# Schatten2021/rust-raytracing

Measured on AMD Instinct MI355X. Metric: Mrays/s (primary rays, whole node), 10k-sphere 1080p 64spp, higher is better.
Workload: dtype f64; 1 GPU; C2: 10k random spheres (scene seed 1), 1920x1080, 64 spp; width=1920, height=1080, rays_per_pixel=64, n_objects=10000, partition=single GPU

## Files before the change

### rust-raytracing_amd/csrc/rtx_bvh.h

```cpp
#pragma once

#include <hip/hip_runtime.h>
#include <stdint.h>

#include <algorithm>
#include <cmath>
#include <cstring>
#include <numeric>
#include <vector>

namespace rtx {

struct BvhNode {
    float lo[3];
    uint32_t link;
    float hi[3];
    uint32_t count;
};
static_assert(sizeof(BvhNode) == 32, "BvhNode must be 32 bytes");

constexpr uint32_t kBvhTriLeaf = 0x10000u;
constexpr int kBvhLeafSize = 1;
constexpr int kBvhTriLeafMax = 8;

struct BvhBox { double lo[3], hi[3]; };

struct BvhBuild {
    std::vector<BvhNode> nodes;
    std::vector<uint32_t> prims;
    std::vector<uint32_t> tri_order;
    std::vector<uint8_t> flat;
    bool has_spheres = false, has_tris = false;
    double origin_limit = 0.0;
    double abs_pad = 0.0;
};

inline float round_down_f32(double x)
{
    float f = (float)x;
    if ((double)f > x) f = std::nextafterf(f, -INFINITY);
    return f;
}

inline float round_up_f32(double x)
{
    float f = (float)x;
    if ((double)f < x) f = std::nextafterf(f, INFINITY);
    return f;
}

inline bool sphere_box(const double s[4], BvhBox &b)
{
    const double r = std::fabs(s[3]);
    for (int a = 0; a < 3; ++a) {
        if (!std::isfinite(s[a]) || !std::isfinite(r)) return false;
        const double pad = (std::fabs(s[a]) + r) * (1.0 / 1048576.0) + 1e-300;
        b.lo[a] = s[a] - r - pad;
        b.hi[a] = s[a] + r + pad;
    }
    return true;
}

inline bool triangle_footprint(const double v[9], BvhBox &b, int free_axis = 2)
{
    for (int a = 0; a < 3; ++a) {
        if (a == free_axis) { b.lo[a] = -INFINITY; b.hi[a] = INFINITY; continue; }
        const double x0 = v[a], x1 = v[3 + a], x2 = v[6 + a];
        if (!std::isfinite(x0) || !std::isfinite(x1) || !std::isfinite(x2)) return false;
        const double lo = std::fmin(x0, std::fmin(x1, x2)), hi = std::fmax(x0, std::fmax(x1, x2));
        const double pad = std::fmax(std::fabs(lo), std::fabs(hi)) * (1.0 / 1048576.0) + 1e-300;
        b.lo[a] = lo - pad;
        b.hi[a] = hi + pad;
    }
    return true;
}

#ifndef RTX_BVH_SAH_BINS
#define RTX_BVH_SAH_BINS 16
#endif
constexpr int kBvhSahBins = RTX_BVH_SAH_BINS;
constexpr int kBvhSahExtraDepth = 6;

inline void bvh_append_tree(const std::vector<BvhBox> &box, int dims, uint32_t leaf_size, uint32_t leaf_flag,
                            BvhBuild &out, std::vector<uint32_t> &order_out, bool use_sah = true, int free_axis = 2,
                            uint32_t order_base = 0)
{
    const uint32_t n = (uint32_t)box.size();
    const int ax[3] = { dims == 2 && free_axis == 0 ? 1 : 0, dims == 2 && free_axis != 2 ? 2 : 1, 2 };
    std::vector<double> cen((size_t)dims * n);
    for (uint32_t i = 0; i < n; ++i)
        for (int a = 0; a < dims; ++a) cen[(size_t)dims * i + a] = 0.5 * (box[i].lo[ax[a]] + box[i].hi[ax[a]]);
    std::vector<uint32_t> order(n);
    std::iota(order.begin(), order.end(), 0u);
    int balanced_depth = 1;
    for (uint64_t c = leaf_size; c < n; c *= 2) ++balanced_depth;
    const int max_depth = balanced_depth + kBvhSahExtraDepth;
    auto measure = [dims, &ax](const BvhBox &b) {
        const double dx = b.hi[ax[0]] - b.lo[ax[0]], dy = b.hi[ax[1]] - b.lo[ax[1]];
        if (dims == 2) return dx + dy;
        const double dz = b.hi[2] - b.lo[2];
        return dx * dy + dy * dz + dz * dx;
    };
    auto grow = [](BvhBox &b, const BvhBox &o) {
        for (int a = 0; a < 3; ++a) { b.lo[a] = std::min(b.lo[a], o.lo[a]); b.hi[a] = std::max(b.hi[a], o.hi[a]); }
    };
    auto empty_box = [] {
        BvhBox b;
        for (int a = 0; a < 3; ++a) { b.lo[a] = INFINITY; b.hi[a] = -INFINITY; }
        return b;
    };
    struct Task { uint32_t begin, end; int parent; int depth; };
    std::vector<Task> todo;
    todo.push_back({0u, n, -1, 1});
    while (!todo.empty()) {
        const Task t = todo.back();
        todo.pop_back();
        const uint32_t me = (uint32_t)out.nodes.size();
        if (t.parent >= 0) out.nodes[(size_t)t.parent].link = me;
        BvhBox b = empty_box();
        double clo[3], chi[3];
        for (int a = 0; a < 3; ++a) { clo[a] = INFINITY; chi[a] = -INFINITY; }
        for (uint32_t k = t.begin; k < t.end; ++k) {
            const uint32_t i = order[k];
            grow(b, box[i]);
            for (int a = 0; a < dims; ++a) {
                clo[a] = std::min(clo[a], cen[(size_t)dims * i + a]); chi[a] = std::max(chi[a], cen[(size_t)dims * i + a]);
            }
        }
        BvhNode node;
        for (int a = 0; a < 3; ++a) {
            node.lo[a] = round_down_f32(b.lo[a] - out.abs_pad);
            node.hi[a] = round_up_f32(b.hi[a] + out.abs_pad);
        }
        const uint32_t cnt = t.end - t.begin;
        if (cnt <= leaf_size) {
            node.link = (uint32_t)order_out.size();
            node.count = cnt | leaf_flag;
            for (uint32_t k = t.begin; k < t.end; ++k) order_out.push_back(order_base + order[k]);
            out.nodes.push_back(node);
            continue;
        }
        uint32_t mid = 0;
        bool sah_allowed = use_sah && cnt > 2;
        if (sah_allowed) {
            int need = 1;
            for (uint64_t c = leaf_size; c < cnt; c *= 2) ++need;
            sah_allowed = t.depth + need < max_depth;
        }
        if (sah_allowed) {
            double best_cost = INFINITY;
            int best_axis = -1, best_bin = -1;
            for (int a = 0; a < dims; ++a) {
                const double ext = chi[a] - clo[a];
                if (!(ext > 0.0)) continue;
                BvhBox bin_box[kBvhSahBins];
                uint32_t bin_cnt[kBvhSahBins];
                for (int k = 0; k < kBvhSahBins; ++k) { bin_box[k] = empty_box(); bin_cnt[k] = 0; }
                const double scale = (double)kBvhSahBins / ext;
                for (uint32_t k = t.begin; k < t.end; ++k) {
                    const uint32_t i = order[k];
                    int bi = (int)((cen[(size_t)dims * i + a] - clo[a]) * scale);
                    bi = bi < 0 ? 0 : (bi >= kBvhSahBins ? kBvhSahBins - 1 : bi);
                    grow(bin_box[bi], box[i]);
                    bin_cnt[bi] += 1;
                }
                double right_m[kBvhSahBins];
                uint32_t right_n[kBvhSahBins];
                BvhBox acc = empty_box();
                uint32_t accn = 0;
                for (int k = kBvhSahBins - 1; k >= 1; --k) {
                    if (bin_cnt[k]) grow(acc, bin_box[k]);
                    accn += bin_cnt[k];
                    right_m[k] = accn ? measure(acc) : 0.0;
                    right_n[k] = accn;
                }
                acc = empty_box();
                accn = 0;
                for (int k = 0; k + 1 < kBvhSahBins; ++k) {
                    if (bin_cnt[k]) grow(acc, bin_box[k]);
                    accn += bin_cnt[k];
                    if (accn == 0 || right_n[k + 1] == 0) continue;
                    const double cost = measure(acc) * accn + right_m[k + 1] * right_n[k + 1];
                    if (cost < best_cost) { best_cost = cost; best_axis = a; best_bin = k; }
                }
            }
            if (best_axis >= 0) {
                const double ext = chi[best_axis] - clo[best_axis];
                const double scale = (double)kBvhSahBins / ext;
                auto in_left = [&](uint32_t i) {
                    int bi = (int)((cen[(size_t)dims * i + best_axis] - clo[best_axis]) * scale);
                    bi = bi < 0 ? 0 : (bi >= kBvhSahBins ? kBvhSahBins - 1 : bi);
                    return bi <= best_bin;
                };
                mid = (uint32_t)(std::stable_partition(order.begin() + t.begin, order.begin() + t.end, in_left) - order.begin());
            }
        }
        if (mid <= t.begin || mid >= t.end) {
            int axis = 0;
            for (int a = 1; a < dims; ++a)
                if (chi[a] - clo[a] > chi[axis] - clo[axis]) axis = a;
            mid = t.begin + cnt / 2;
            std::nth_element(order.begin() + t.begin, order.begin() + mid, order.begin() + t.end,
                             [&](uint32_t x, uint32_t y) {
                                 const double cx = cen[(size_t)dims * x + axis], cy = cen[(size_t)dims * y + axis];
                                 return cx < cy || (cx == cy && x < y);
                             });
        }
        node.link = 0;
        node.count = 0;
        out.nodes.push_back(node);
        todo.push_back({mid, t.end, (int)me, t.depth + 1});
        todo.push_back({t.begin, mid, -1, t.depth + 1});
    }
}

inline BvhBuild build_bvh(const std::vector<BvhBox> &sphere_boxes, const std::vector<BvhBox> (&tri_boxes)[3], uint32_t tri_leaf_size,
                          bool use_sah = true)
{
    BvhBuild out;
    const bool want_s = !sphere_boxes.empty();
    const size_t n_tri = tri_boxes[0].size() + tri_boxes[1].size() + tri_boxes[2].size();
    if (!want_s && n_tri == 0) return out;
    double scale = 0.0;
    auto grow_scale = [&](const std::vector<BvhBox> &v) {
        for (const BvhBox &b : v)
            for (int a = 0; a < 3; ++a) {
                if (std::isfinite(b.lo[a])) scale = std::max(scale, std::fabs(b.lo[a]));
                if (std::isfinite(b.hi[a])) scale = std::max(scale, std::fabs(b.hi[a]));
            }
    };
    grow_scale(sphere_boxes);
    for (const auto &v : tri_boxes) grow_scale(v);
    out.origin_limit = 4.0 * scale + 1.0;
    out.abs_pad = out.origin_limit * (1.0 / 4194304.0);
    if (!(out.origin_limit < 1.0e28)) return BvhBuild();
    if (sphere_boxes.size() + n_tri >= 0x10000000ull) return BvhBuild();
    if (tri_leaf_size < 1) tri_leaf_size = 1;
    if (tri_leaf_size > (uint32_t)kBvhTriLeafMax) tri_leaf_size = (uint32_t)kBvhTriLeafMax;
    out.nodes.reserve(2 * (sphere_boxes.size() + n_tri) + 8);
    struct Sub { const std::vector<BvhBox> *boxes; int free_axis; uint32_t base; };
    std::vector<Sub> subs;
    if (want_s) subs.push_back({&sphere_boxes, -1, 0u});
    uint32_t base = 0;
    for (int f = 2; f >= 0; --f) {
        if (!tri_boxes[f].empty()) subs.push_back({&tri_boxes[f], f, base});
        base += (uint32_t)tri_boxes[f].size();
    }
    std::vector<uint32_t> joints;
    for (size_t k = 0; k < subs.size(); ++k) {
        if (k + 1 < subs.size()) {
            joints.push_back((uint32_t)out.nodes.size());
            out.nodes.emplace_back();
        } else if (!joints.empty()) {
            out.nodes[joints.back()].link = (uint32_t)out.nodes.size();
        }
        if (k > 0 && k + 1 < subs.size()) out.nodes[joints[k - 1]].link = joints[k];
        const size_t first = out.nodes.size();
        if (subs[k].free_axis < 0) {
            bvh_append_tree(*subs[k].boxes, 3, (uint32_t)kBvhLeafSize, 0u, out, out.prims, use_sah);
            out.has_spheres = true;
        } else {
            bvh_append_tree(*subs[k].boxes, 2, tri_leaf_size, kBvhTriLeaf, out, out.tri_order, use_sah, subs[k].free_axis, subs[k].base);
            out.has_tris = true;
        }
        out.flat.resize(out.nodes.size(), 0);
        if (subs[k].free_axis == 2) std::fill(out.flat.begin() + (ptrdiff_t)first, out.flat.end(), (uint8_t)1);
    }
    for (size_t k = joints.size(); k-- > 0;) {
        BvhNode &j = out.nodes[joints[k]];
        const BvhNode &l = out.nodes[joints[k] + 1], &r = out.nodes[j.link];
        for (int a = 0; a < 3; ++a) { j.lo[a] = std::min(l.lo[a], r.lo[a]); j.hi[a] = std::max(l.hi[a], r.hi[a]); }
        j.count = 0;
    }
    return out;
}

struct Bvh4Node {
    float4 a[4];
    float4 b[4];
};
static_assert(sizeof(Bvh4Node) == 128, "Bvh4Node must be 128 bytes");

#ifndef RTX_BVH_STACK
#define RTX_BVH_STACK 30
#endif
constexpr int kBvh4StackEntries = RTX_BVH_STACK;

constexpr uint32_t kBvhFlatNode = 0x80000000u;

struct Bvh4Build {
    std::vector<Bvh4Node> nodes;
    int depth = 0;
    uint32_t root = 0;
};

inline float u32_as_f32(uint32_t u) { float f; std::memcpy(&f, &u, 4); return f; }
constexpr int kBvhTopLevels = 6;

inline Bvh4Build collapse_to_bvh4(const BvhBuild &b2)
{
    Bvh4Build out;
    if (b2.nodes.empty()) return out;
    auto area = [&](uint32_t i) {
        const BvhNode &n = b2.nodes[i];
        double e[3], fin[3];
        int nf = 0;
        for (int a = 0; a < 3; ++a) { e[a] = (double)n.hi[a] - n.lo[a]; if (std::isfinite(e[a])) fin[nf++] = e[a]; }
        if (nf == 3) return e[0] * e[1] + e[1] * e[2] + e[2] * e[0];
        if (nf == 2) return fin[0] + fin[1];
        return (double)INFINITY;
    };
    auto flat = [&](uint32_t bin) { return bin < b2.flat.size() && b2.flat[bin] != 0; };
    struct Task { uint32_t bin; uint32_t wide; int depth; };
    std::vector<Task> todo, top;
    size_t top_head = 0;
    out.nodes.emplace_back();
    out.root = flat(0u) ? kBvhFlatNode : 0u;
    top.push_back({0u, 0u, 1});
    while (top_head < top.size() || !todo.empty()) {
        Task t;
        if (top_head < top.size()) t = top[top_head++];
        else { t = todo.back(); todo.pop_back(); }
        out.depth = std::max(out.depth, t.depth);
        uint32_t kids[4];
        int nk = 0;
        if (b2.nodes[t.bin].count != 0) {
            kids[nk++] = t.bin;
        } else {
            kids[nk++] = t.bin + 1;
            kids[nk++] = b2.nodes[t.bin].link;
            while (nk < 4) {
                int best = -1;
                double best_area = -1.0;
                for (int k = 0; k < nk; ++k)
                    if (b2.nodes[kids[k]].count == 0 && area(kids[k]) > best_area) { best = k; best_area = area(kids[k]); }
                if (best < 0) break;
                const uint32_t open = kids[best];
                kids[best] = open + 1;
                kids[nk++] = b2.nodes[open].link;
            }
        }
        Bvh4Node w;
        const bool wflat = flat(t.bin);
        uint32_t links[4] = { 0u, 0u, 0u, 0u }, counts[4] = { 0xFFFFFFFFu, 0xFFFFFFFFu, 0xFFFFFFFFu, 0xFFFFFFFFu };
        for (int c = 0; c < 4; ++c) {
            if (c < nk) {
                const BvhNode &n = b2.nodes[kids[c]];
                uint32_t link = n.link, count = n.count;
                if (count == 0) {
                    link = (uint32_t)out.nodes.size();
                    out.nodes.emplace_back();
                    (t.depth + 1 <= kBvhTopLevels ? top : todo).push_back({kids[c], link, t.depth + 1});
                    if (flat(kids[c])) link |= kBvhFlatNode;
                }
                links[c] = link; counts[c] = count;
                if (wflat) w.a[c] = make_float4(n.lo[0], n.lo[1], n.hi[0], n.hi[1]);
                else {
                    w.a[c] = make_float4(n.lo[0], n.lo[1], n.lo[2], u32_as_f32(link));
                    w.b[c] = make_float4(n.hi[0], n.hi[1], n.hi[2], u32_as_f32(count));
                }
            } else if (wflat) {
                w.a[c] = make_float4(INFINITY, INFINITY, -INFINITY, -INFINITY);
            } else {
                w.a[c] = make_float4(INFINITY, INFINITY, INFINITY, u32_as_f32(0u));
                w.b[c] = make_float4(-INFINITY, -INFINITY, -INFINITY, u32_as_f32(0xFFFFFFFFu));
            }
        }
        if (wflat) {
            w.b[0] = make_float4(u32_as_f32(links[0]), u32_as_f32(links[1]), u32_as_f32(links[2]), u32_as_f32(links[3]));
            w.b[1] = make_float4(u32_as_f32(counts[0]), u32_as_f32(counts[1]), u32_as_f32(counts[2]), u32_as_f32(counts[3]));
            w.b[2] = make_float4(0.f, 0.f, 0.f, 0.f);
            w.b[3] = make_float4(0.f, 0.f, 0.f, 0.f);
        }
        out.nodes[t.wide] = w;
    }
    return out;
}

constexpr uint32_t kQNodeShift = 29, kQNodeIndexMask = (1u << 29) - 1u, kQNodeEmpty = 7u, kQNodeLeafMax = 6u;
struct BvhQNode {
    float ox, oy, sx, sy;
    uint32_t qx[4], qy[4], link[4];
};
static_assert(sizeof(BvhQNode) == 64, "BvhQNode must be 64 bytes");

inline bool build_qnodes(const Bvh4Build &b4, std::vector<BvhQNode> &out)
{
    out.clear();
    out.reserve(b4.nodes.size());
    auto bits = [](float f) { uint32_t u; std::memcpy(&u, &f, 4); return u; };
    for (const Bvh4Node &w : b4.nodes) {
        const uint32_t lk[4] = { bits(w.b[0].x), bits(w.b[0].y), bits(w.b[0].z), bits(w.b[0].w) };
        const uint32_t ct[4] = { bits(w.b[1].x), bits(w.b[1].y), bits(w.b[1].z), bits(w.b[1].w) };
        double lo[2] = { INFINITY, INFINITY }, hi[2] = { -INFINITY, -INFINITY };
        for (int c = 0; c < 4; ++c) {
            if (ct[c] == 0xFFFFFFFFu) continue;
            const float r[4] = { w.a[c].x, w.a[c].y, w.a[c].z, w.a[c].w };
            for (int k = 0; k < 4; ++k) if (!std::isfinite(r[k])) return false;
            lo[0] = std::min(lo[0], (double)r[0]); lo[1] = std::min(lo[1], (double)r[1]);
            hi[0] = std::max(hi[0], (double)r[2]); hi[1] = std::max(hi[1], (double)r[3]);
        }
        BvhQNode q;
        double o[2], sc[2];
        for (int a = 0; a < 2; ++a) {
            o[a] = std::isfinite(lo[a]) ? lo[a] : 0.0;
            const double ext = std::isfinite(lo[a]) ? hi[a] - lo[a] : 0.0;
            sc[a] = ext > 0.0 ? std::exp2(std::ceil(std::log2(ext / 65535.0))) : 1.0;
            while (ext / sc[a] > 65535.0) sc[a] *= 2.0;
            if (!(sc[a] >= 1.1754944e-38 && sc[a] <= 1.0e30)) return false;
        }
        q.ox = (float)o[0]; q.oy = (float)o[1]; q.sx = (float)sc[0]; q.sy = (float)sc[1];
        for (int c = 0; c < 4; ++c) {
            if (ct[c] == 0xFFFFFFFFu) { q.qx[c] = 0x0000FFFFu; q.qy[c] = 0x0000FFFFu; q.link[c] = kQNodeEmpty << kQNodeShift; continue; }
            const double l0 = std::floor(((double)w.a[c].x - o[0]) / sc[0]), h0 = std::ceil(((double)w.a[c].z - o[0]) / sc[0]);
            const double l1 = std::floor(((double)w.a[c].y - o[1]) / sc[1]), h1 = std::ceil(((double)w.a[c].w - o[1]) / sc[1]);
            if (l0 < 0 || l1 < 0 || h0 > 65535 || h1 > 65535) return false;
            q.qx[c] = (uint32_t)l0 | ((uint32_t)h0 << 16);
            q.qy[c] = (uint32_t)l1 | ((uint32_t)h1 << 16);
            uint32_t type;
            if (ct[c] == 0u) type = 0u;
            else if ((ct[c] & kBvhTriLeaf) && (ct[c] & 0xFFFFu) >= 1u && (ct[c] & 0xFFFFu) <= kQNodeLeafMax) type = ct[c] & 0xFFFFu;
            else return false;
            const uint32_t idx = lk[c] & ~kBvhFlatNode;
            if (idx > kQNodeIndexMask) return false;
            if (type == 0u && !(lk[c] & kBvhFlatNode)) return false;
            q.link[c] = (type << kQNodeShift) | idx;
        }
        out.push_back(q);
    }
    return true;
}


struct BvhQ3Node {
    float ox, oy, oz, sx;
    float sy, sz;
    uint32_t lox, loy;
    uint32_t loz, hix, hiy, hiz;
    uint32_t link[4];
};
static_assert(sizeof(BvhQ3Node) == 64, "BvhQ3Node must be 64 bytes");

inline bool build_q3nodes(const Bvh4Build &b4, double abs_pad, std::vector<BvhQ3Node> &out)
{
    out.clear();
    out.reserve(b4.nodes.size());
    auto bits = [](float f) { uint32_t u; std::memcpy(&u, &f, 4); return u; };
    for (const Bvh4Node &w : b4.nodes) {
        double lo[3] = { INFINITY, INFINITY, INFINITY }, hi[3] = { -INFINITY, -INFINITY, -INFINITY };
        uint32_t cnt[4], lnk[4];
        for (int c = 0; c < 4; ++c) {
            cnt[c] = bits(w.b[c].w); lnk[c] = bits(w.a[c].w);
            if (cnt[c] == 0xFFFFFFFFu) continue;
            const float l[3] = { w.a[c].x, w.a[c].y, w.a[c].z }, h[3] = { w.b[c].x, w.b[c].y, w.b[c].z };
            for (int a = 0; a < 3; ++a) {
                if (!std::isfinite(l[a]) || !std::isfinite(h[a])) return false;
                lo[a] = std::min(lo[a], (double)l[a] - abs_pad); hi[a] = std::max(hi[a], (double)h[a] + abs_pad);
            }
        }
        BvhQ3Node q;
        std::memset(&q, 0, sizeof q);
        double o[3], sc[3];
        for (int a = 0; a < 3; ++a) {
            const double ext = std::isfinite(lo[a]) ? hi[a] - lo[a] : 0.0;
            sc[a] = ext > 0.0 ? std::exp2(std::ceil(std::log2(ext / 254.0))) : 1.0;
            if (!(sc[a] >= 1.1754944e-38 && sc[a] <= 1.0e30)) return false;
            o[a] = std::isfinite(lo[a]) ? std::floor(lo[a] / sc[a]) * sc[a] : 0.0;
            while (std::isfinite(lo[a]) && (hi[a] - o[a]) / sc[a] > 255.0) { sc[a] *= 2.0; o[a] = std::floor(lo[a] / sc[a]) * sc[a]; }
            if (!(std::fabs(o[a] / sc[a]) + 256.0 < 16777216.0)) return false;
            if ((double)(float)o[a] != o[a]) return false;
        }
        q.ox = (float)o[0]; q.oy = (float)o[1]; q.oz = (float)o[2]; q.sx = (float)sc[0]; q.sy = (float)sc[1]; q.sz = (float)sc[2];
        uint32_t *lows[3] = { &q.lox, &q.loy, &q.loz }, *highs[3] = { &q.hix, &q.hiy, &q.hiz };
        for (int c = 0; c < 4; ++c) {
            if (cnt[c] == 0xFFFFFFFFu) {
                for (int a = 0; a < 3; ++a) *lows[a] |= 255u << (8 * c);
                q.link[c] = kQNodeEmpty << kQNodeShift;
                continue;
            }
            const float l[3] = { w.a[c].x, w.a[c].y, w.a[c].z }, h[3] = { w.b[c].x, w.b[c].y, w.b[c].z };
            for (int a = 0; a < 3; ++a) {
                const double ql = std::floor(((double)l[a] - abs_pad - o[a]) / sc[a]), qh = std::ceil(((double)h[a] + abs_pad - o[a]) / sc[a]);
                if (ql < 0 || qh > 255 || ql > qh) return false;
                *lows[a] |= (uint32_t)ql << (8 * c);
                *highs[a] |= (uint32_t)qh << (8 * c);
            }
            uint32_t type;
            if (cnt[c] == 0u) type = 0u;
            else if ((cnt[c] & kBvhTriLeaf) == 0u && cnt[c] >= 1u && cnt[c] <= kQNodeLeafMax) type = cnt[c];
            else return false;
            if (lnk[c] > kQNodeIndexMask || (lnk[c] & kBvhFlatNode)) return false;
            q.link[c] = (type << kQNodeShift) | lnk[c];
        }
        out.push_back(q);
    }
    return true;
}

}
```

Before: 3601 Mrays/s.

## Constrain BVH4 collapse height so traversal stack fits in LDS for spheres

Adds a dynamic-programming pass that computes the minimum achievable 4-wide tree height per binary node, and uses it during BVH2-to-BVH4 collapse to pick child groupings that keep total depth within a level budget derived from the traversal stack size. If the SAH tree is too deep, the sphere tree is rebuilt with a tighter extra-depth limit. It also adds optional full-sweep SAH and cost-optimal collapse, both disabled by default. The intent is to bound traversal depth so a small stack, possibly in LDS, always suffices, at the cost of slightly worse SAH quality and more host build time.

```diff
diff --git a/rust-raytracing_amd/csrc/rtx_bvh.h b/rust-raytracing_amd/csrc/rtx_bvh.h
--- a/rust-raytracing_amd/csrc/rtx_bvh.h
+++ b/rust-raytracing_amd/csrc/rtx_bvh.h
@@ -81,9 +81,53 @@
 constexpr int kBvhSahBins = RTX_BVH_SAH_BINS;
 constexpr int kBvhSahExtraDepth = 6;
 
+#ifndef RTX_BVH_STACK
+#define RTX_BVH_STACK 30
+#endif
+constexpr int kBvh4StackEntries = RTX_BVH_STACK;
+constexpr int kBvhLdsLevels = (kBvh4StackEntries - 2) / 3;
+#ifndef RTX_BVH_FIT_LDS
+#define RTX_BVH_FIT_LDS 1
+#endif
+struct BvhHeights { std::vector<uint8_t> low[5], open[5]; };
+inline void bvh_least_heights(const std::vector<BvhNode> &nodes, BvhHeights &h)
+{
+    const size_t n2 = nodes.size();
+    for (int k = 1; k <= 4; ++k) { h.low[k].assign(n2, 0); h.open[k].assign(n2, 0); }
+    for (size_t v = n2; v-- > 0;) {
+        const BvhNode &n = nodes[v];
+        if (n.count != 0) continue;
+        const size_t l = v + 1, r = n.link;
+        int split[5];
+        uint8_t left[5];
+        split[1] = 255; left[1] = 0;
+        for (int k = 2; k <= 4; ++k) {
+            split[k] = split[k - 1]; left[k] = left[k - 1];
+            for (int i = 1; i < k; ++i) {
+                const int c = std::max((int)h.low[i][l], (int)h.low[k - i][r]);
+                if (c < split[k]) { split[k] = c; left[k] = (uint8_t)i; }
+            }
+        }
+        const int own = std::min(split[4] + 1, 255);
+        h.low[1][v] = (uint8_t)own; h.open[1][v] = left[4];
+        for (int k = 2; k <= 4; ++k) {
+            if (split[k] < own) { h.low[k][v] = (uint8_t)split[k]; h.open[k][v] = left[k]; }
+            else { h.low[k][v] = (uint8_t)own; h.open[k][v] = 0; }
+        }
+    }
+}
+
+#ifndef RTX_BVH_SPHERE_BUILD
+#define RTX_BVH_SPHERE_BUILD 0
+#endif
+#ifndef RTX_BVH_SWEEP_BELOW
+#define RTX_BVH_SWEEP_BELOW 512
+#endif
+constexpr uint32_t kBvhSweepBelow = RTX_BVH_SPHERE_BUILD >= 2 ? RTX_BVH_SWEEP_BELOW : 0;
+
 inline void bvh_append_tree(const std::vector<BvhBox> &box, int dims, uint32_t leaf_size, uint32_t leaf_flag,
                             BvhBuild &out, std::vector<uint32_t> &order_out, bool use_sah = true, int free_axis = 2,
-                            uint32_t order_base = 0)
+                            uint32_t order_base = 0, uint32_t sweep_below = 0, int extra_depth = kBvhSahExtraDepth)
 {
     const uint32_t n = (uint32_t)box.size();
     const int ax[3] = { dims == 2 && free_axis == 0 ? 1 : 0, dims == 2 && free_axis != 2 ? 2 : 1, 2 };
@@ -94,7 +138,7 @@
     std::iota(order.begin(), order.end(), 0u);
     int balanced_depth = 1;
     for (uint64_t c = leaf_size; c < n; c *= 2) ++balanced_depth;
-    const int max_depth = balanced_depth + kBvhSahExtraDepth;
+    const int max_depth = balanced_depth + extra_depth;
     auto measure = [dims, &ax](const BvhBox &b) {
         const double dx = b.hi[ax[0]] - b.lo[ax[0]], dy = b.hi[ax[1]] - b.lo[ax[1]];
         if (dims == 2) return dx + dy;
@@ -111,6 +155,8 @@
     };
     struct Task { uint32_t begin, end; int parent; int depth; };
     std::vector<Task> todo;
+    std::vector<uint32_t> sweep_idx, sweep_best;
+    std::vector<double> sweep_right;
     todo.push_back({0u, n, -1, 1});
     while (!todo.empty()) {
         const Task t = todo.back();
@@ -147,7 +193,33 @@
             for (uint64_t c = leaf_size; c < cnt; c *= 2) ++need;
             sah_allowed = t.depth + need < max_depth;
         }
-        if (sah_allowed) {
+        if (sah_allowed && cnt <= sweep_below) {
+            double best_cost = INFINITY;
+            int best_axis = -1;
+            uint32_t best_k = 0;
+            for (int a = 0; a < dims; ++a) {
+                if (!(chi[a] - clo[a] > 0.0)) continue;
+                sweep_idx.assign(order.begin() + t.begin, order.begin() + t.end);
+                std::sort(sweep_idx.begin(), sweep_idx.end(), [&](uint32_t x, uint32_t y) {
+                    const double cx = cen[(size_t)dims * x + a], cy = cen[(size_t)dims * y + a];
+                    return cx < cy || (cx == cy && x < y);
+                });
+                sweep_right.resize(cnt);
+                BvhBox acc = empty_box();
+                for (uint32_t k = cnt; k-- > 1;) { grow(acc, box[sweep_idx[k]]); sweep_right[k] = measure(acc); }
+                acc = empty_box();
+                for (uint32_t k = 1; k < cnt; ++k) {
+                    grow(acc, box[sweep_idx[k - 1]]);
+                    const double cost = measure(acc) * k + sweep_right[k] * (cnt - k);
+                    if (cost < best_cost) { best_cost = cost; best_axis = a; best_k = k; }
+                }
+                if (best_axis == a) sweep_best = sweep_idx;
+            }
+            if (best_axis >= 0) {
+                std::copy(sweep_best.begin(), sweep_best.end(), order.begin() + t.begin);
+                mid = t.begin + best_k;
+            }
+        } else if (sah_allowed) {
             double best_cost = INFINITY;
             int best_axis = -1, best_bin = -1;
             for (int a = 0; a < dims; ++a) {
@@ -257,7 +329,21 @@
         if (k > 0 && k + 1 < subs.size()) out.nodes[joints[k - 1]].link = joints[k];
         const size_t first = out.nodes.size();
         if (subs[k].free_axis < 0) {
-            bvh_append_tree(*subs[k].boxes, 3, (uint32_t)kBvhLeafSize, 0u, out, out.prims, use_sah);
+            bvh_append_tree(*subs[k].boxes, 3, (uint32_t)kBvhLeafSize, 0u, out, out.prims, use_sah, 2, 0u,
+                            n_tri == 0 ? kBvhSweepBelow : 0u);
+            if (RTX_BVH_FIT_LDS && n_tri == 0 && use_sah) {
+                int balanced = 1;
+                for (uint64_t c = (uint64_t)kBvhLeafSize; c < sphere_boxes.size(); c *= 2) ++balanced;
+                const int sure = 2 * kBvhLdsLevels + 1 - balanced;
+                BvhHeights hts;
+                for (int extra = sure + 1; extra >= sure && sure >= 0; --extra) {
+                    if (extra >= kBvhSahExtraDepth) continue;
+                    bvh_least_heights(out.nodes, hts);
+                    if ((int)hts.low[1][0] <= kBvhLdsLevels) break;
+                    out.nodes.clear(); out.prims.clear();
+                    bvh_append_tree(*subs[k].boxes, 3, (uint32_t)kBvhLeafSize, 0u, out, out.prims, use_sah, 2, 0u, kBvhSweepBelow, extra);
+                }
+            }
             out.has_spheres = true;
         } else {
             bvh_append_tree(*subs[k].boxes, 2, tri_leaf_size, kBvhTriLeaf, out, out.tri_order, use_sah, subs[k].free_axis, subs[k].base);
@@ -281,10 +367,6 @@
 };
 static_assert(sizeof(Bvh4Node) == 128, "Bvh4Node must be 128 bytes");
 
-#ifndef RTX_BVH_STACK
-#define RTX_BVH_STACK 30
-#endif
-constexpr int kBvh4StackEntries = RTX_BVH_STACK;
 
 constexpr uint32_t kBvhFlatNode = 0x80000000u;
 
@@ -311,6 +393,57 @@
         return (double)INFINITY;
     };
     auto flat = [&](uint32_t bin) { return bin < b2.flat.size() && b2.flat[bin] != 0; };
+    constexpr double kLeafCost = 70.0 / 125.0;
+    const size_t n2 = b2.nodes.size();
+    const bool optimal = RTX_BVH_SPHERE_BUILD >= 1 && b2.has_spheres && !b2.has_tris;
+    std::vector<double> cut[5];
+    std::vector<uint8_t> open[5];
+    if (optimal) {
+        for (int k = 1; k <= 4; ++k) { cut[k].assign(n2, 0.0); open[k].assign(n2, 0); }
+        for (size_t v = n2; v-- > 0;) {
+            const BvhNode &n = b2.nodes[v];
+            if (n.count != 0) {
+                for (int k = 1; k <= 4; ++k) cut[k][v] = kLeafCost * area((uint32_t)v) * (double)(n.count & 0xFFFFu);
+                continue;
+            }
+            const size_t l = v + 1, r = n.link;
+            double split[5];
+            uint8_t left[5];
+            split[1] = INFINITY; left[1] = 0;
+            for (int k = 2; k <= 4; ++k) {
+                split[k] = split[k - 1]; left[k] = left[k - 1];
+                for (int i = 1; i < k; ++i) {
+                    const double c = cut[i][l] + cut[k - i][r];
+                    if (c < split[k]) { split[k] = c; left[k] = (uint8_t)i; }
+                }
+            }
+            cut[1][v] = area((uint32_t)v) + split[4];
+            open[1][v] = left[4];
+            for (int k = 2; k <= 4; ++k) {
+                if (split[k] < cut[1][v]) { cut[k][v] = split[k]; open[k][v] = left[k]; }
+                else { cut[k][v] = cut[1][v]; open[k][v] = 0; }
+            }
+        }
+    }
+    BvhHeights hts;
+    int levels = 1 << 30;
+    if (RTX_BVH_FIT_LDS && b2.has_spheres && !b2.has_tris) {
+        bvh_least_heights(b2.nodes, hts);
+        if ((int)hts.low[1][0] <= kBvhLdsLevels) levels = kBvhLdsLevels;
+    }
+    const std::vector<uint8_t> (&low)[5] = hts.low, (&low_open)[5] = hts.open;
+    auto expand = [&](const std::vector<uint8_t> (&op)[5], uint32_t u0, int k0, uint32_t *kids, int &nk) {
+        struct Part { uint32_t u; int k; } st[8];
+        int ns = 0;
+        st[ns++] = { u0, k0 };
+        while (ns > 0) {
+            const Part p = st[--ns];
+            if (b2.nodes[p.u].count != 0 || p.k == 1 || op[p.k][p.u] == 0) { kids[nk++] = p.u; continue; }
+            const int li = op[p.k][p.u];
+            st[ns++] = { b2.nodes[p.u].link, p.k - li };
+            st[ns++] = { p.u + 1, li };
+        }
+    };
     struct Task { uint32_t bin; uint32_t wide; int depth; };
     std::vector<Task> todo, top;
     size_t top_head = 0;
@@ -326,6 +459,10 @@
         int nk = 0;
         if (b2.nodes[t.bin].count != 0) {
             kids[nk++] = t.bin;
+        } else if (optimal) {
+            const int li = open[1][t.bin];
+            expand(open, t.bin + 1, li, kids, nk);
+            expand(open, b2.nodes[t.bin].link, 4 - li, kids, nk);
         } else {
             kids[nk++] = t.bin + 1;
             kids[nk++] = b2.nodes[t.bin].link;
@@ -338,6 +475,17 @@
                 const uint32_t open = kids[best];
                 kids[best] = open + 1;
                 kids[nk++] = b2.nodes[open].link;
+            }
+        }
+        if (levels < (1 << 30)) {
+            bool fits = true;
+            for (int k = 0; k < nk; ++k)
+                if (b2.nodes[kids[k]].count == 0 && (int)low[1][kids[k]] > levels - t.depth) fits = false;
+            if (!fits) {
+                const int li = low_open[1][t.bin];
+                nk = 0;
+                expand(low_open, t.bin + 1, li, kids, nk);
+                expand(low_open, b2.nodes[t.bin].link, 4 - li, kids, nk);
             }
         }
         Bvh4Node w;
```

Measured after the change: 3599 Mrays/s (median of 3 runs). Within noise of the previous version (-0.1%).
